# schwanbeck/YSMR

Measured on AMD Instinct MI355X. Metric: frames/sec detect+link, 1228x922 ~500 blobs, 1/2/4/8 GPU; HBM GB/s %peak, higher is better.
Workload: dtype u8 image / f32 threshold+geometry / f64 link; 1 GPU; 1228x922 stream, ~500 blobs, detect+link end to end (BASELINE configs[2], the configuration the metric is quoted on); detect_batch=248, channels=1, streams=1, parallelism=1 stream/GPU x1, tracks_alive=508, ids_issued=796

## Files before the change

ysmr_amd/csrc/batch_link.h:

```cpp
#pragma once

#include "tracker_plan.h"

constexpr unsigned BL_FLAG = 0xFFFFu, BL_SPLIT = 0xFFFEu;

constexpr int BG_THREADS = 256, BG_PER = 10;
constexpr int BG_CAND = 32;
static_assert(BG_THREADS == 4 * 64 && BL_OVF <= 64, "k_bgrid's second pass: quadrant w of overflow entry `lane` on wave w");
static_assert(BG_THREADS * BG_PER >= FUSED_MAX_DET, "k_bgrid keeps a frame's detections in registers, BG_PER per thread");

__device__ __forceinline__ void bl_rect_list(int cx, int cy, float ax, float bx, float ay, float by, float e, int G, int m, float cell,
                                             float inv, const unsigned short *start16, const float2 *xy, unsigned short *list8,
                                             unsigned short *cand)
{
    float u2 = 3.0e38f;
    int ju = 0;
    auto far2 = [&](int a, int b) {
        for (int j = a; j < b; ++j) {
            const float2 d = xy[j];
            const float dx = fmaxf(fabsf(d.x - ax), fabsf(d.x - bx)), dy = fmaxf(fabsf(d.y - ay), fabsf(d.y - by));
            const float v = dx * dx + dy * dy;
            ju = v < u2 ? j : ju;
            u2 = fminf(u2, v);
        }
    };
    for (int r = 0; r < G; ++r) {
        const int xl = max(cx - r, 0), xh = min(cx + r, G - 1);
        for (int y = max(cy - r, 0); y <= min(cy + r, G - 1); ++y) {
            if (y == cy - r || y == cy + r) far2(start16[y * G + xl], start16[y * G + xh + 1]);
            else {
                if (cx - r >= 0) far2(start16[y * G + cx - r], start16[y * G + cx - r + 1]);
                if (cx + r < G) far2(start16[y * G + cx + r], start16[y * G + cx + r + 1]);
            }
        }
        const float reach = (float)(r + 1) * cell;
        if (u2 <= reach * reach) break;
    }
    const float T = sqrtf(u2) * 1.0001f + 1.0f, T2 = T * T;
    const int rho = min((int)((T + e) * inv) + 2, G);
    int n = 0;
    for (int y = max(cy - rho, 0); y <= min(cy + rho, G - 1); ++y) {
        const int a = start16[y * G + max(cx - rho, 0)], b = start16[y * G + min(cx + rho, G - 1) + 1];
        for (int j = a; j < b; ++j) {
            const float2 d = xy[j];
            const float dx = fmaxf(fmaxf(ax - d.x, d.x - bx), 0.f), dy = fmaxf(fmaxf(ay - d.y, d.y - by), 0.f);
            if (dx * dx + dy * dy <= T2) {
                if (n < BG_CAND) cand[n * BG_THREADS] = (unsigned short)j;
                ++n;
            }
        }
    }
    int kept = 0;
    const float2 du = xy[ju];
    const float ua = ax - du.x, ub = bx - du.x, va = ay - du.y, vb = by - du.y;
    const float eps = 1.00003f, beta = 0.6f;
    const float u0 = (ua * ua + va * va) * eps + beta, u1 = (ub * ub + va * va) * eps + beta;
    const float u2c = (ua * ua + vb * vb) * eps + beta, u3 = (ub * ub + vb * vb) * eps + beta;
    if (n <= BG_CAND)
        for (int i = 0; i < n; ++i) {
            const int ji = cand[i * BG_THREADS];
            const float2 di = xy[ji];
            const float xa = ax - di.x, xb = bx - di.x, ya = ay - di.y, yb = by - di.y;
            const float s0 = xa * xa + ya * ya, s1 = xb * xb + ya * ya, s2 = xa * xa + yb * yb, s3 = xb * xb + yb * yb;
            bool beaten = ji != ju && s0 > u0 && s1 > u1 && s2 > u2c && s3 > u3;
            for (int k = 0; k < n && !beaten; k += 4) {
                float2 dk[4];
#pragma unroll
                for (int u = 0; u < 4; ++u) dk[u] = xy[cand[min(k + u, n - 1) * BG_THREADS]];
#pragma unroll
                for (int u = 0; u < 4; ++u) {
                    const float ka = ax - dk[u].x, kb = bx - dk[u].x, la = ay - dk[u].y, lb = by - dk[u].y;
                    beaten = beaten || (k + u < n && k + u != i && s0 > (ka * ka + la * la) * eps + beta && s1 > (kb * kb + la * la) * eps + beta &&
                                        s2 > (ka * ka + lb * lb) * eps + beta && s3 > (kb * kb + lb * lb) * eps + beta);
                }
            }
            if (!beaten) {
                if (kept < BL_LIST) list8[kept] = (unsigned short)ji;
                ++kept;
            }
        }
    if (n > BG_CAND || kept > BL_LIST) list8[0] = (unsigned short)BL_FLAG;
    else
        for (int k = kept; k < BL_LIST; ++k) list8[k] = (unsigned short)m;
}
__device__ __forceinline__ void bl_cell_list(int c, int G, int m, float x0, float y0, float cell, float inv, const unsigned short *start16,
                                             const float2 *xy, unsigned short *list16, unsigned short *cand)
{
    const int cx = c % G, cy = c / G;
    const float e = 4e-3f + 2e-4f * cell;
    const float ax = x0 + (float)cx * cell - e, bx = x0 + (float)(cx + 1) * cell + e;
    const float ay = y0 + (float)cy * cell - e, by = y0 + (float)(cy + 1) * cell + e;
    bl_rect_list(cx, cy, ax, bx, ay, by, e, G, m, cell, inv, start16, xy, list16 + c * BL_LIST, cand);
}
__device__ __forceinline__ void bl_quad_list(int c, int q, int G, int m, float x0, float y0, float cell, float inv, const unsigned short *start16,
                                             const float2 *xy, unsigned short *list8, unsigned short *cand)
{
    const int cx = c % G, cy = c / G;
    const float e = 4e-3f + 2e-4f * cell;
    const float hx = (float)cx + 0.5f * (float)(q & 1), hy = (float)cy + 0.5f * (float)(q >> 1);
    const float ax = x0 + hx * cell - e, bx = x0 + (hx + 0.5f) * cell + e;
    const float ay = y0 + hy * cell - e, by = y0 + (hy + 0.5f) * cell + e;
    bl_rect_list(cx, cy, ax, bx, ay, by, e, G, m, cell, inv, start16, xy, list8, cand);
}

template <bool D3>
__device__ __forceinline__ void bl_bin_frame(const float *__restrict__ det_all, const double *__restrict__ third_all,
                                             const int32_t *__restrict__ det_count, int max_det, char *grid, unsigned grid_stride)
{
    extern __shared__ __attribute__((aligned(16))) uint32_t s_out[];
    __shared__ int s_cnt[64 * 64];
    __shared__ float s_red[4][4];
    __shared__ int s_wave_sum[4];
    const int f = blockIdx.x, tid = threadIdx.x, lane = tid & 63, w = tid >> 6;
    __shared__ unsigned short s_cand[BG_CAND][BG_THREADS];
    __shared__ unsigned short s_crowded[BL_OVF];
    __shared__ int s_crowded_n;
    __shared__ int s_any_crowded;
    __shared__ int s_wide;
    const float *det = det_all + (size_t)f * max_det * 5;
    int m = det_count[f];
    m = m < 0 ? 0 : (m > max_det ? max_det : m);
    const int G = bl_grid_n(m), cells = G * G;
    unsigned short *start16 = reinterpret_cast<unsigned short *>(s_out + 16);
    float2 *xy = reinterpret_cast<float2 *>(s_out + 16 + bl_start_dwords(G));
    unsigned short *items = reinterpret_cast<unsigned short *>(s_out + 16 + bl_start_dwords(G) + 2 * bl_mp(m));
    unsigned short *list16 = reinterpret_cast<unsigned short *>(s_out + bl_list_off(m));
    float *z32 = reinterpret_cast<float *>(s_out + bl_list_off(m));
    double *z64 = nullptr;
    if constexpr (D3) z64 = reinterpret_cast<double *>(grid + (size_t)grid_stride * f + 4 * (size_t)bl3_lds_dwords_max(max_det));
    float x[BG_PER], y[BG_PER];
    double z[BG_PER];
    bool wide = false;
#pragma unroll
    for (int k = 0; k < BG_PER; ++k) {
        const int j = tid + k * BG_THREADS;
        x[k] = j < m ? det[(size_t)j * 5] : 0.f;
        y[k] = j < m ? det[(size_t)j * 5 + 1] : 0.f;
        if constexpr (D3) {
            z[k] = j < m ? (third_all + (size_t)f * max_det)[j] : 0.0;
            wide = wide || !(fabs(z[k]) < 4096.0);
        }
    }
    for (int c = tid; c < cells; c += BG_THREADS) s_cnt[c] = 0;
    if constexpr (D3) { if (tid == 0) s_wide = 0; }
    float lo_x = 3.0e38f, lo_y = 3.0e38f, hi_x = -3.0e38f, hi_y = -3.0e38f;
#pragma unroll
    for (int k = 0; k < BG_PER; ++k)
        if (tid + k * BG_THREADS < m) { lo_x = fminf(lo_x, x[k]); hi_x = fmaxf(hi_x, x[k]); lo_y = fminf(lo_y, y[k]); hi_y = fmaxf(hi_y, y[k]); }
#pragma unroll
    for (int d = 32; d >= 1; d >>= 1) {
        lo_x = fminf(lo_x, __shfl_xor(lo_x, d)); hi_x = fmaxf(hi_x, __shfl_xor(hi_x, d));
        lo_y = fminf(lo_y, __shfl_xor(lo_y, d)); hi_y = fmaxf(hi_y, __shfl_xor(hi_y, d));
    }
    if (lane == 0) { s_red[0][w] = lo_x; s_red[1][w] = hi_x; s_red[2][w] = lo_y; s_red[3][w] = hi_y; }
    __syncthreads();
    if constexpr (D3) { if (wide) s_wide = 1; }
    lo_x = s_red[0][0]; hi_x = s_red[1][0]; lo_y = s_red[2][0]; hi_y = s_red[3][0];
    for (int k = 1; k < 4; ++k) {
        lo_x = fminf(lo_x, s_red[0][k]); hi_x = fmaxf(hi_x, s_red[1][k]);
        lo_y = fminf(lo_y, s_red[2][k]); hi_y = fmaxf(hi_y, s_red[3][k]);
    }
    if (m == 0) { lo_x = lo_y = 0.f; hi_x = hi_y = 1.f; }
    const float extent = fmaxf(fmaxf(hi_x - lo_x, hi_y - lo_y), 1.0f);
    const float cell = extent / (float)(G - 2), inv = 1.0f / cell;
    const float x0 = lo_x - cell, y0 = lo_y - cell;
    if (tid < 16) s_out[tid] = 0;
    __syncthreads();
    if (tid == 0) {
        float *h = reinterpret_cast<float *>(s_out);
        h[0] = x0; h[1] = y0; h[2] = cell; h[3] = inv;
        s_out[4] = (uint32_t)G; s_out[5] = (uint32_t)m; s_out[6] = !D3 && bl_has_lists(m) ? BL_LIST : 0;
        if constexpr (D3) s_out[7] = (uint32_t)s_wide;
    }
    int cell_of[BG_PER];
#pragma unroll
    for (int k = 0; k < BG_PER; ++k) {
        int cx = (int)floorf((x[k] - x0) * inv), cy = (int)floorf((y[k] - y0) * inv);
        cx = cx < 0 ? 0 : (cx > G - 1 ? G - 1 : cx);
        cy = cy < 0 ? 0 : (cy > G - 1 ? G - 1 : cy);
        cell_of[k] = cy * G + cx;
        if (tid + k * BG_THREADS < m) atomicAdd(&s_cnt[cell_of[k]], 1);
    }
    __syncthreads();
    const int K = cells / BG_THREADS;
    int local[16], sum = 0;
#pragma unroll
    for (int k = 0; k < 16; ++k)
        if (k < K) { local[k] = sum; sum += s_cnt[tid * K + k]; }
    int incl = sum;
#pragma unroll
    for (int d = 1; d < 64; d <<= 1) { const int o = __shfl_up(incl, d); if (lane >= d) incl += o; }
    if (lane == 63) s_wave_sum[w] = incl;
    __syncthreads();
    int before = incl - sum;
    for (int k = 0; k < w; ++k) before += s_wave_sum[k];
#pragma unroll
    for (int k = 0; k < 16; ++k)
        if (k < K) {
            const int at = before + local[k];
            s_cnt[tid * K + k] = at;
            start16[tid * K + k] = (unsigned short)at;
        }
    if (tid == BG_THREADS - 1) { start16[cells] = (unsigned short)m; start16[cells + 1] = 0; }
    for (int j = m + tid; j < bl_mp(m); j += BG_THREADS) {
        xy[j] = make_float2(1.0e30f, 1.0e30f); items[j] = 0;
        if constexpr (D3) { z32[j] = 0.f; z64[j] = 0.0; }
    }
    __syncthreads();
#pragma unroll
    for (int k = 0; k < BG_PER; ++k) {
        const int j = tid + k * BG_THREADS;
        if (j < m) {
            const int at = atomicAdd(&s_cnt[cell_of[k]], 1);
            items[at] = (unsigned short)j;
            xy[at] = make_float2(x[k], y[k]);
            if constexpr (D3) { z32[at] = (float)z[k]; z64[at] = z[k]; }
        }
    }
    if (!D3 && bl_has_lists(m)) {
        for (int i = tid; i < BL_OVF * 4 * BL_LIST / 2; i += BG_THREADS) s_out[bl_ovf_off(m) + i] = 0;
        if (tid == 0) s_any_crowded = 0;
    }
    __syncthreads();
    if constexpr (!D3) {
        unsigned short *ovf16 = reinterpret_cast<unsigned short *>(s_out + bl_ovf_off(m));
        if (bl_has_lists(m) && m > 0) {
            for (int c = tid; c < cells; c += BG_THREADS) {
                bl_cell_list(c, G, m, x0, y0, cell, inv, start16, xy, list16, &s_cand[0][tid]);
                if (list16[c * BL_LIST] == BL_FLAG) s_any_crowded = 1;
            }
            __syncthreads();
        }
        if (bl_has_lists(m) && m > 0 && s_any_crowded) {
            int mine = 0;
#pragma unroll
            for (int k = 0; k < 16; ++k)
                if (k < K) mine += list16[(tid * K + k) * BL_LIST] == BL_FLAG;
            int inc2 = mine;
#pragma unroll
            for (int d = 1; d < 64; d <<= 1) { const int o = __shfl_up(inc2, d); if (lane >= d) inc2 += o; }
            if (lane == 63) s_wave_sum[w] = inc2;
            __syncthreads();
            int at = inc2 - mine;
            for (int k = 0; k < w; ++k) at += s_wave_sum[k];
            if (mine)
                for (int k = 0; k < K; ++k)
                    if (list16[(tid * K + k) * BL_LIST] == BL_FLAG) {
                        if (at < BL_OVF) s_crowded[at] = (unsigned short)(tid * K + k);
                        ++at;
                    }
            if (tid == BG_THREADS - 1) s_crowded_n = min(at, BL_OVF);
            __syncthreads();
            const int entries = s_crowded_n;
            if (lane < entries)
                bl_quad_list(s_crowded[lane], w, G, m, x0, y0, cell, inv, start16, xy, ovf16 + (4 * lane + w) * BL_LIST, &s_cand[0][tid]);
            __syncthreads();
            if (tid < entries) {
                bool fits = true;
                for (int q = 0; q < 4; ++q) fits = fits && ovf16[(4 * tid + q) * BL_LIST] != BL_FLAG;
                if (fits) reinterpret_cast<uint32_t *>(list16)[s_crowded[tid] * (BL_LIST / 2)] = BL_SPLIT | ((uint32_t)tid << 16);
            }
            __syncthreads();
        }
    }
    uint4 *out = reinterpret_cast<uint4 *>(grid + (size_t)grid_stride * f);
    const uint4 *img = reinterpret_cast<const uint4 *>(s_out);
    for (int i = tid; i < (D3 ? bl3_lds_dwords(m) : bl_grid_dwords(m)) / 4; i += BG_THREADS) out[i] = img[i];
}

__global__ __launch_bounds__(BG_THREADS) void k_bgrid(const float *__restrict__ det_all, const int32_t *__restrict__ det_count,
                                                      int max_det, char *grid, unsigned grid_stride)
{
    bl_bin_frame<false>(det_all, nullptr, det_count, max_det, grid, grid_stride);
}

struct BlSeat {
    double s0x[BL_NF], s1x[BL_NF], s0y[BL_NF], s1y[BL_NF];
    double w[BL_NF], xa[BL_NF], xb[BL_NF];
    double px, py;
    float info[3];
    int id, gone, len, mode, rank;
    bool alive;
};

__device__ __forceinline__ void bl_seat_blank(BlSeat &S)
{
#pragma unroll
    for (int f = 0; f < BL_NF; ++f) { S.s0x[f] = S.s1x[f] = S.s0y[f] = S.s1y[f] = 0.0; S.w[f] = S.xa[f] = S.xb[f] = 0.0; }
    S.px = S.py = 0.0;
    S.info[0] = S.info[1] = S.info[2] = 0.f;
    S.id = S.gone = S.len = S.mode = S.rank = 0;
    S.alive = false;
}

__device__ __forceinline__ void bl_seat_load(BlSeat &S, const BatchDev &bd, int at)
{
    const size_t sc = (size_t)bd.seat_cap;
    const double *p = bd.f64 + at;
#pragma unroll
    for (int f = 0; f < BL_NF; ++f) { S.w[f] = p[sc * f]; S.xa[f] = p[sc * (BL_NF + f)]; S.xb[f] = p[sc * (2 * BL_NF + f)]; }
    S.px = p[sc * (3 * BL_NF)];
    S.py = p[sc * (3 * BL_NF + 1)];
#pragma unroll
    for (int f = 0; f < BL_NF; ++f) {
        const double *q = p + sc * (3 * BL_NF + 2 + 4 * f);
        S.s0x[f] = q[0]; S.s1x[f] = q[sc]; S.s0y[f] = q[2 * sc]; S.s1y[f] = q[3 * sc];
    }
#pragma unroll
    for (int k = 0; k < 3; ++k) S.info[k] = bd.f32[sc * k + at];
    S.id = bd.i32[at]; S.gone = bd.i32[sc + at]; S.len = bd.i32[2 * sc + at]; S.mode = bd.i32[3 * sc + at];
    S.rank = bd.i32[4 * sc + at];
}

__device__ __forceinline__ void bl_seat_store(const BlSeat &S, const BatchDev &bd, int at)
{
    const size_t sc = (size_t)bd.seat_cap;
    double *p = bd.f64 + at;
#pragma unroll
    for (int f = 0; f < BL_NF; ++f) { p[sc * f] = S.w[f]; p[sc * (BL_NF + f)] = S.xa[f]; p[sc * (2 * BL_NF + f)] = S.xb[f]; }
    p[sc * (3 * BL_NF)] = S.px;
    p[sc * (3 * BL_NF + 1)] = S.py;
#pragma unroll
    for (int f = 0; f < BL_NF; ++f) {
        double *q = p + sc * (3 * BL_NF + 2 + 4 * f);
        q[0] = S.s0x[f]; q[sc] = S.s1x[f]; q[2 * sc] = S.s0y[f]; q[3 * sc] = S.s1y[f];
    }
#pragma unroll
    for (int k = 0; k < 3; ++k) bd.f32[sc * k + at] = S.info[k];
    bd.i32[at] = S.id; bd.i32[sc + at] = S.gone; bd.i32[2 * sc + at] = S.len; bd.i32[3 * sc + at] = S.mode;
    bd.i32[4 * sc + at] = S.rank;
}

__device__ __forceinline__ double2 bl_ring_load(const BatchDev &bd, int pos, int seat)
{
    const double *p = reinterpret_cast<const double *>(bd.ring + (size_t)pos * bd.seat_cap + seat);
    double2 v;
    v.x = __hip_atomic_load(p, __ATOMIC_RELAXED, __HIP_MEMORY_SCOPE_AGENT);
    v.y = __hip_atomic_load(p + 1, __ATOMIC_RELAXED, __HIP_MEMORY_SCOPE_AGENT);
    return v;
}
__device__ __forceinline__ double2 bl_ring_load_bytes(const BatchDev &bd, unsigned at)
{
    const double *p = reinterpret_cast<const double *>(reinterpret_cast<const char *>(bd.ring) + at);
    double2 v;
    v.x = __hip_atomic_load(p, __ATOMIC_RELAXED, __HIP_MEMORY_SCOPE_AGENT);
    v.y = __hip_atomic_load(p + 1, __ATOMIC_RELAXED, __HIP_MEMORY_SCOPE_AGENT);
    return v;
}
typedef uint32_t bl_u32x4 __attribute__((ext_vector_type(4)));
__device__ __forceinline__ bl_u32x4 bl_ring_load16(const double2 *p)
{
    bl_u32x4 v;
    asm volatile("global_load_dwordx4 %0, %1, off sc1\n\ts_waitcnt vmcnt(0)" : "=&v"(v) : "v"(p) : "memory");
    return v;
}
constexpr int BL_RING_GROUP = 3;
// ... 1653 lines not shown
```

ysmr_amd/csrc/track.hip:

```cpp
#include "common.h"
#include "set_order.h"
#include "tracker_plan.h"
#include <algorithm>
#include <cmath>
#include <cstdlib>
#include <cstring>
#include <vector>

struct DetGrid {
    const int *start;
    const int *items;
    const float *hdr;
    const float2 *xy;
};

namespace plan = tracker_plan;

struct ysmr_tracker {
    TrackerDev d;
    TrackerDev d1;
    int par = 0;
    plan::Config cfg;
    plan::Caps caps;
    int dims = 2;
// ... 1922 lines not shown
int ysmr_debug_read_bcounts(unsigned long long *out) { return (int)hipMemcpyFromSymbol(out, HIP_SYMBOL(g_bcounts), sizeof(unsigned long long) * BL_WAVES * BL_COUNTS); }
int ysmr_debug_read_bwaves(unsigned long long *out) { return (int)hipMemcpyFromSymbol(out, HIP_SYMBOL(g_bwaves), sizeof(unsigned long long) * (BL_WAVES + 1)); }
int ysmr_debug_read_bseats(unsigned long long *out) { return (int)hipMemcpyFromSymbol(out, HIP_SYMBOL(g_bseats), sizeof(unsigned long long) * 2); }
int ysmr_debug_read_brefresh(unsigned long long *out) { return (int)hipMemcpyFromSymbol(out, HIP_SYMBOL(g_brefresh), sizeof(unsigned long long) * BL_WAVES * 4); }
int ysmr_debug_read_bsteady(unsigned long long *out) { return (int)hipMemcpyFromSymbol(out, HIP_SYMBOL(g_bsteady), sizeof(unsigned long long) * BL_WAVES * 16); }
#endif

int ysmr_tracker_batched(ysmr_tracker *t) { return t && plan::is_batch(t->link()) ? 1 : 0; }

int ysmr_debug_ring_poison(ysmr_tracker *t)
{
    if (!t) return ysmr::fail(YSMR_ERR_ARG, "tracker handle is NULL");
    hipError_t e = hipDeviceSynchronize();
    int seen[2] = {0, 0};
    if (e == hipSuccess) e = hipMemcpy(seen, t->cur().n_tracks, sizeof(seen), hipMemcpyDeviceToHost);
    if (e == hipSuccess && (seen[0] != 0 || seen[1] != 0))
        return ysmr::fail(YSMR_ERR_ARG, "ysmr_debug_ring_poison is for a handle that has held no track yet");
    if (e == hipSuccess) e = hipMemset(t->bd.ring, 0xFF, sizeof(double2) * BL_HB * (size_t)t->bd.seat_cap);
    if (e == hipSuccess) e = hipDeviceSynchronize();
    return e == hipSuccess ? YSMR_OK : ysmr::fail(YSMR_ERR_HIP, "ring poison failed: %s", hipGetErrorString(e));
}
static int seat_words(ysmr_tracker *t, int (&w)[3])
{
    if (!t) return ysmr::fail(YSMR_ERR_ARG, "tracker handle is NULL");
    hipError_t e = hipDeviceSynchronize();
    if (e == hipSuccess) e = hipMemcpy(w, t->bd.head + 1, sizeof(w), hipMemcpyDeviceToHost);
    return e == hipSuccess ? YSMR_OK : ysmr::fail(YSMR_ERR_HIP, "seat words read failed: %s", hipGetErrorString(e));
}
int ysmr_debug_seat_events(ysmr_tracker *t, int *events_out, int *moved_out)
{
    int w[3];
    if (!events_out || !moved_out) return ysmr::fail(YSMR_ERR_ARG, "events_out and moved_out must be set");
    if (int rc = seat_words(t, w)) return rc;
    *events_out = w[0]; *moved_out = w[1];
    return YSMR_OK;
}
int ysmr_debug_track_waves(ysmr_tracker *t, int *out)
{
    int w[3];
    if (!out) return ysmr::fail(YSMR_ERR_ARG, "out must be set");
    if (int rc = seat_words(t, w)) return rc;
    *out = w[2];
    return YSMR_OK;
}
int ysmr_debug_ring_zero_line(ysmr_tracker *t, long long *nonzero)
{
    if (!t || !nonzero) return ysmr::fail(YSMR_ERR_ARG, "tracker handle and nonzero must be set");
    std::vector<unsigned long long> line(2 * (size_t)t->bd.seat_cap);
    hipError_t e = hipDeviceSynchronize();
    if (e == hipSuccess)
        e = hipMemcpy(line.data(), t->bd.ring + (size_t)BL_HB * t->bd.seat_cap, sizeof(double2) * (size_t)t->bd.seat_cap, hipMemcpyDeviceToHost);
    if (e != hipSuccess) return ysmr::fail(YSMR_ERR_HIP, "ring read failed: %s", hipGetErrorString(e));
    *nonzero = 0;
    for (unsigned long long w : line) *nonzero += w != 0;
    return YSMR_OK;
}

int ysmr_debug_read_grid_block(ysmr_tracker *t, int slot, int frame, void *out, size_t bytes)
{
    if (!t || !out) return ysmr::fail(YSMR_ERR_ARG, "tracker handle and out must be set");
    if (t->link() != plan::Link::batch) return ysmr::fail(YSMR_ERR_STATE, "the handle has no batch link: no grid blocks");
    if (slot < 0 || slot > 1 || t->prepared[slot].batch <= 0 || frame < 0 || frame >= t->prepared[slot].batch || bytes > t->bd.grid_stride)
        return ysmr::fail(YSMR_ERR_ARG, "slot 0 or 1 with a prepared batch, a frame of that batch, at most %u bytes", t->bd.grid_stride);
    hipError_t e = hipDeviceSynchronize();
    if (e == hipSuccess)
        e = hipMemcpy(out, t->bd.grid + ((size_t)slot * BL_MAX_BATCH + (size_t)frame) * t->bd.grid_stride, bytes, hipMemcpyDeviceToHost);
    return e == hipSuccess ? YSMR_OK : ysmr::fail(YSMR_ERR_HIP, "grid block read failed: %s", hipGetErrorString(e));
}

static BatchDev batch_dev(const ysmr_tracker *t, int block)
{
    BatchDev bd = t->bd;
    if (t->dims == 3) { bd.grid = (char *)t->grid3_block; bd.grid_stride = t->grid3_stride; }
    bd.grid += (size_t)block * BL_MAX_BATCH * bd.grid_stride;
    return bd;
}

static void bin_batch(const ysmr_tracker *t, hipStream_t st, const float *det, const double *third, const int32_t *count, int batch,
                      const BatchDev &bd)
{
    if (t->dims == 3)
        hipLaunchKernelGGL(k_bgrid3, dim3(batch), dim3(BG_THREADS), 4 * (size_t)bl3_lds_dwords_max(t->d.max_det), st, det, third, count,
                           t->d.max_det, bd.grid, bd.grid_stride);
    else
        hipLaunchKernelGGL(k_bgrid, dim3(batch), dim3(BG_THREADS), bd.grid_stride, st, det, count, t->d.max_det, bd.grid, bd.grid_stride);
}

static int tracker_prepare(ysmr_tracker *t, hipStream_t st, const float *det_dev, const double *third_dev, const int32_t *det_count_dev,
                           int batch, int slot)
{
    if (!plan::is_batch(t->link()) || batch > BL_MAX_BATCH) return YSMR_OK;
    bin_batch(t, st, det_dev, third_dev, det_count_dev, batch, batch_dev(t, slot));
    YSMR_LAUNCH_CHECK();
    t->prepared[slot] = ysmr_tracker::Prepared{det_dev, det_count_dev, third_dev, batch};
    return YSMR_OK;
}

int ysmr_tracker_prepare(ysmr_tracker *t, void *stream, const float *det_dev, const int32_t *det_count_dev, int batch, int slot)
{
    if (!t) return ysmr::fail(YSMR_ERR_ARG, "tracker handle is NULL");
    if (!det_dev || !det_count_dev || batch <= 0 || slot < 0 || slot > 1)
        return ysmr::fail(YSMR_ERR_ARG, "det_dev, det_count_dev must be set, batch > 0, slot 0 or 1");
    if (t->dims != 2) return YSMR_OK;
    return tracker_prepare(t, (hipStream_t)stream, det_dev, nullptr, det_count_dev, batch, slot);
}

int ysmr_tracker_prepare3(ysmr_tracker *t, void *stream, const float *det_dev, const double *third_dev, const int32_t *det_count_dev,
                          int batch, int slot)
{
    if (!t) return ysmr::fail(YSMR_ERR_ARG, "tracker handle is NULL");
    if (!det_dev || !third_dev || !det_count_dev || batch <= 0 || slot < 0 || slot > 1)
        return ysmr::fail(YSMR_ERR_ARG, "det_dev, third_dev, det_count_dev must be set, batch > 0, slot 0 or 1");
    if (t->dims != 3) return ysmr::fail(YSMR_ERR_STATE, "ysmr_tracker_prepare3 needs a 3-D handle (ysmr_tracker_dimensions)");
    return tracker_prepare(t, (hipStream_t)stream, det_dev, third_dev, det_count_dev, batch, slot);
}

static int tracker_update(ysmr_tracker *t, hipStream_t st, const void *det_dev, int det_is_f64, const double *third_dev, int m,
                          const int32_t *m_dev, int32_t frame_index, ysmr_row *rows_dev, int32_t *n_rows_dev, int32_t *claim_col_dev,
                          int32_t *n_before_dev, int32_t *new_cols_dev, int32_t *n_new_dev)
{
    if (int rc = state_to_std(t, st)) return rc;
    FrameArgs a;
    a.det = det_dev; a.f64 = det_is_f64 != 0; a.third = third_dev;
    a.m = m; a.m_dev = m_dev; a.frame = frame_index;
    a.rows = rows_dev; a.rows_capacity = t->d.capacity;
    a.n_rows = n_rows_dev; a.claim = claim_col_dev; a.n_before = n_before_dev; a.new_cols = new_cols_dev; a.n_new = n_new_dev;
    return launch_frame(t, st, a);
}

int ysmr_tracker_update(ysmr_tracker *t, void *stream, const void *det_dev, int det_is_f64, int m,
                        const int32_t *m_dev, int32_t frame_index, ysmr_row *rows_dev, int32_t *n_rows_dev,
                        int32_t *claim_col_dev, int32_t *n_before_dev, int32_t *new_cols_dev, int32_t *n_new_dev)
{
    if (!t) return ysmr::fail(YSMR_ERR_ARG, "tracker handle is NULL");
    if (m < 0 && !m_dev) return ysmr::fail(YSMR_ERR_ARG, "m < 0 requires m_dev");
    if (m > t->d.max_det) return ysmr::fail(YSMR_ERR_CAPACITY, "m = %d exceeds max_det = %d", m, t->d.max_det);
    if (!det_dev && m != 0) return ysmr::fail(YSMR_ERR_ARG, "det_dev is NULL");
    if (t->dims != 2) return ysmr::fail(YSMR_ERR_STATE, "a 3-D handle is updated with ysmr_tracker_update3");
    return tracker_update(t, (hipStream_t)stream, det_dev, det_is_f64, nullptr, m, m_dev, frame_index, rows_dev, n_rows_dev,
                          claim_col_dev, n_before_dev, new_cols_dev, n_new_dev);
}

int ysmr_tracker_update3(ysmr_tracker *t, void *stream, const void *det_dev, int det_is_f64, const double *third_dev, int m,
                         const int32_t *m_dev, int32_t frame_index, ysmr_row *rows_dev, int32_t *n_rows_dev,
                         int32_t *claim_col_dev, int32_t *n_before_dev, int32_t *new_cols_dev, int32_t *n_new_dev)
{
    if (!t) return ysmr::fail(YSMR_ERR_ARG, "tracker handle is NULL");
    if (m < 0 && !m_dev) return ysmr::fail(YSMR_ERR_ARG, "m < 0 requires m_dev");
    if (m > t->d.max_det) return ysmr::fail(YSMR_ERR_CAPACITY, "m = %d exceeds max_det = %d", m, t->d.max_det);
    if ((!det_dev || !third_dev) && m != 0) return ysmr::fail(YSMR_ERR_ARG, "det_dev / third_dev is NULL");
    if (t->dims != 3) return ysmr::fail(YSMR_ERR_STATE, "ysmr_tracker_update3 needs a 3-D handle (ysmr_tracker_dimensions)");
    return tracker_update(t, (hipStream_t)stream, det_dev, det_is_f64, third_dev, m, m_dev, frame_index, rows_dev, n_rows_dev,
                          claim_col_dev, n_before_dev, new_cols_dev, n_new_dev);
}

static int tracker_run(ysmr_tracker *t, hipStream_t st, const float *det_dev, const double *third_dev, const int32_t *det_count_dev,
                       int batch, int32_t first_frame_index, ysmr_row *rows_dev, long long rows_capacity, long long *row_count_dev)
{
    const bool d3 = t->dims == 3;
    const size_t md = (size_t)t->d.max_det;
    t->linked = true;
    if (plan::is_batch(t->link())) {
        if (int rc = state_to_batch(t, st)) return rc;
        for (int f0 = 0; f0 < batch; f0 += BL_MAX_BATCH) {
            const int nb = std::min(batch - f0, BL_MAX_BATCH);
            const float *det = det_dev + (size_t)f0 * md * 5;
            const double *third = d3 ? third_dev + (size_t)f0 * md : nullptr;
            int block = 2;
// ... 129 lines not shown
```

ysmr_amd/csrc/tracker_plan.h:

```cpp
#pragma once
#include <cmath>
#include <cstddef>
#include <cstdint>
#include <cstring>
#include <vector>

#include "hd.h"

#ifndef __HIPCC__
struct alignas(16) double2 { double x, y; };
#endif

#define YSMR_MAX_FILTERS 8

struct TrackerDev {
    int *n_tracks, *next_id, *err, *n_free;
    int *order, *gone;
    int *row_arg;
    double *row_min;
    long long *row_base;
    int capacity, max_det, n_f, use_gsff, hist_cap, table_cap, gain_total, gone_by_row;
    int gains_decoupled;
    double max_gone, lik_min;
    int n_i[YSMR_MAX_FILTERS];
// ... 13 lines not shown
    int *set_table;
    unsigned long long *link_key;
    int *link_row;
    int *link_claim;
    int *claim_slot;
    int *claim_row;
};

#ifndef YSMR_BL_THREADS
#define YSMR_BL_THREADS 768
#endif
constexpr int BL_THREADS = YSMR_BL_THREADS;
constexpr int BL_WAVES = BL_THREADS / 64;
constexpr int BL_HB = 32;
constexpr int BL_NF = 3;
#ifndef YSMR_BL_MAX_BATCH
#define YSMR_BL_MAX_BATCH 256
#endif
constexpr int BL_MAX_BATCH = YSMR_BL_MAX_BATCH;
constexpr int BL_TABLE = 4096;
constexpr int BL_SF64 = 3 * BL_NF + 2 + 4 * BL_NF;
constexpr int BL_REFRESH = 64;

struct BatchDev {
    double2 *ring;
    double *f64;
    float *f32;
    int *i32;
    int *head;
    char *grid;
    unsigned grid_stride;
    int seat_cap;
};

struct BlGains { double alpha[BL_NF][2], beta[BL_NF][2]; };
constexpr int GRID_N = 128;
constexpr int GRID_CELLS = GRID_N * GRID_N;
YSMR_HD inline size_t grid_bytes_per_frame(int max_det)
{
    return (sizeof(int) * (GRID_CELLS + 64) + sizeof(int) * (size_t)max_det + 64 + 2 * sizeof(float) * (size_t)max_det + 255) / 256 * 256;
}

constexpr int FRAME_THREADS = 256;
constexpr int FRAME_TABLE = 4096;
YSMR_HD inline size_t frame_lds_bytes(int cap, int max_det, int gain_total)
{
    return 8 * ((size_t)gain_total + max_det) + 4 * ((size_t)max_det + 2 * (size_t)cap + 16) + 2 * 2 * FRAME_TABLE + 64;
}

constexpr int TRACKER_MAX_SIZE = 65536;
constexpr int FUSED_MAX_DET = 2456;
constexpr size_t FRAME_LDS_LIMIT = 150 * 1024;
constexpr double FUSED_MAX_GONE = 32000.0;
constexpr size_t LINK_LDS_LIMIT = 140 * 1024;
constexpr size_t BL_LDS_LIMIT = 160 * 1024;

constexpr int BL_LIST = 8;
constexpr int BL_OVF = 8;
YSMR_HD inline int bl_grid_n(int m) { return m <= 128 ? 16 : (m <= 600 ? 32 : (m <= 1300 ? 48 : 64)); }
YSMR_HD inline bool bl_has_lists(int m) { return bl_grid_n(m) <= 32; }
YSMR_HD inline int bl_start_dwords(int G) { return ((G * G + 2) / 2 + 3) / 4 * 4; }
YSMR_HD inline int bl_pad8(int m) { return (m + 7) / 8 * 8; }
YSMR_HD inline int bl_mp(int m) { return bl_pad8(m + 1); }
YSMR_HD inline int bl_list_off(int m)
{
    return 16 + bl_start_dwords(bl_grid_n(m)) + 2 * bl_mp(m) + bl_mp(m) / 2;
}
YSMR_HD inline int bl_ovf_off(int m)
{
    return bl_list_off(m) + bl_grid_n(m) * bl_grid_n(m) * BL_LIST / 2;
}
YSMR_HD inline int bl_grid_dwords(int m)
{
    const int raw = bl_has_lists(m) ? bl_ovf_off(m) + BL_OVF * 4 * BL_LIST / 2 : bl_list_off(m);
    return (raw + 255) / 256 * 256;
}
YSMR_HD inline int bl_grid_dwords_max(int max_det)
{
    int most = bl_grid_dwords(max_det);
    const int steps[4] = {128, 600, 1300, max_det};
    for (int k = 0; k < 4; ++k)
        if (steps[k] <= max_det && bl_grid_dwords(steps[k]) > most) most = bl_grid_dwords(steps[k]);
    return most;
}

struct BlShared {
    int cnt[BL_MAX_BATCH];
    int used[2];
    int n_dead[2];
    int tie[2];
    int dead_id[2][BL_THREADS];
    int wave_cnt[2][BL_WAVES];
    int set_state[2];
    int top;
    long long rows_then;
};

YSMR_HD inline int bl_md_padded(int max_det) { return (max_det + 3) / 4 * 4; }
YSMR_HD inline size_t bl_lds_bytes(int max_det)
{
    return 2 * 4 * (size_t)bl_grid_dwords_max(max_det) + (3 * 8 + 4) * (size_t)bl_md_padded(max_det) + 4 * BL_TABLE + 64;
}
YSMR_HD inline size_t bl_lds_total(int max_det) { return bl_lds_bytes(max_det) + (sizeof(BlShared) + 15) / 16 * 16; }

YSMR_HD inline int bl3_lds_dwords(int m) { return (bl_list_off(m) + bl_mp(m) + 255) / 256 * 256; }
YSMR_HD inline int bl3_lds_dwords_max(int max_det) { return bl3_lds_dwords(max_det); }
YSMR_HD inline size_t bl3_grid_stride(int max_det)
{
    return 4 * (size_t)bl3_lds_dwords_max(max_det) + (8 * (size_t)bl_mp(max_det) + 1023) / 1024 * 1024;
}
YSMR_HD inline size_t bl3_lds_bytes(int max_det)
{
    return 2 * 4 * (size_t)bl3_lds_dwords_max(max_det) + (3 * 8 + 4) * (size_t)bl_md_padded(max_det) + 4 * BL_TABLE + 64;
}
YSMR_HD inline size_t bl3_lds_total(int max_det) { return bl3_lds_bytes(max_det) + (sizeof(BlShared) + 15) / 16 * 16; }

namespace tracker_plan {

enum class Bad { none, size, filters, fps, horizons, horizon_max };
struct Status {
    Bad what = Bad::none;
    int a = 0, b = 0, c = 0;
    double x = 0.0;
    explicit operator bool() const { return what != Bad::none; }
};

inline Status horizons(double fps, int n_min, double n_max, int n_f, int *n_i)
{
    if (n_f < 1 || n_f > YSMR_MAX_FILTERS) return Status{Bad::filters, YSMR_MAX_FILTERS, n_f};
    if (!(fps > 0)) return Status{Bad::fps};
    double top = n_max > 0 ? n_max : fps;
    double p = (top - n_min) / n_f;
    for (int i = 1; i <= n_f; ++i) n_i[i - 1] = (int)(n_min + p * i);
    for (int i = 0; i < n_f; ++i)
        if (n_i[i] < 1 || (i && n_i[i] <= n_i[i - 1])) return Status{Bad::horizons, n_min, n_f, 0, top};
    return Status{};
}

inline void closed_form_gain(int N, double *g)
{
    double st2 = 0.0;
    for (int j = 0; j < N; ++j) { double tj = j - (N - 1) / 2.0; st2 += tj * tj; }
    std::memset(g, 0, sizeof(double) * 4 * N);
    for (int j = 0; j < N; ++j) {
        double tj = j - (N - 1) / 2.0;
        double c = 1.0 / N + (st2 > 0 ? tj * ((N + 1) / 2.0) / st2 : 0.0);
        g[2 * j] = c;
        g[2 * N + 2 * j + 1] = c;
    }
}

struct Config {
    int capacity, max_det, use_gsff;
    double max_gone;
    int n_f, n_i[YSMR_MAX_FILTERS], gain_off[YSMR_MAX_FILTERS], gain_total;
    int hist_cap, table_cap, rec_stride;
    int gains_decoupled;
    bool gains_affine;
    BlGains bgains;
};

inline Status configure(double max_disappeared, double fps, int n_min, double n_max, int n_f, int use_gsff, int capacity,
                        int max_det, const double *gains, Config &c, std::vector<double> &gains_out)
{
    if (capacity <= 0 || max_det <= 0 || capacity > TRACKER_MAX_SIZE || max_det > TRACKER_MAX_SIZE)
        return Status{Bad::size, capacity, max_det};
// ... 164 lines not shown
```

Before: 293,100 frames/s.

## Split grid binning into bin, per-cell list, and crowded-split kernels

The single per-frame binning kernel used to also build per-cell candidate lists and quadrant overflow lists inside one 256-thread block. This moves list building into k_blist, which launches several blocks per frame (one per 256 cells, with launch bounds allowing four blocks per CU), and moves the crowded-cell quadrant split into k_bsplit, which exits early when no cell is flagged. The aim is more parallelism and less LDS per block than the monolithic kernel allowed. In exchange there are two extra launches per batch and a round trip of the frame's grid through global memory, and the groups and LDS sizes are capped at the m=600 configuration.

Result: no change. 293,600 frames/s, median of 2 (+0.2%).

```diff
diff --git a/ysmr_amd/csrc/batch_link.h b/ysmr_amd/csrc/batch_link.h
--- a/ysmr_amd/csrc/batch_link.h
+++ b/ysmr_amd/csrc/batch_link.h
@@ -6,7 +6,7 @@
 
 constexpr int BG_THREADS = 256, BG_PER = 10;
 constexpr int BG_CAND = 32;
-static_assert(BG_THREADS == 4 * 64 && BL_OVF <= 64, "k_bgrid's second pass: quadrant w of overflow entry `lane` on wave w");
+static_assert(BG_THREADS == 4 * 64 && BL_OVF <= 64, "k_bsplit, the second pass: quadrant w of overflow entry `lane` on wave w");
 static_assert(BG_THREADS * BG_PER >= FUSED_MAX_DET, "k_bgrid keeps a frame's detections in registers, BG_PER per thread");
 
 __device__ __forceinline__ void bl_rect_list(int cx, int cy, float ax, float bx, float ay, float by, float e, int G, int m, float cell,
@@ -84,13 +84,13 @@
         for (int k = kept; k < BL_LIST; ++k) list8[k] = (unsigned short)m;
 }
 __device__ __forceinline__ void bl_cell_list(int c, int G, int m, float x0, float y0, float cell, float inv, const unsigned short *start16,
-                                             const float2 *xy, unsigned short *list16, unsigned short *cand)
+                                             const float2 *xy, unsigned short *list8, unsigned short *cand)
 {
     const int cx = c % G, cy = c / G;
     const float e = 4e-3f + 2e-4f * cell;
     const float ax = x0 + (float)cx * cell - e, bx = x0 + (float)(cx + 1) * cell + e;
     const float ay = y0 + (float)cy * cell - e, by = y0 + (float)(cy + 1) * cell + e;
-    bl_rect_list(cx, cy, ax, bx, ay, by, e, G, m, cell, inv, start16, xy, list16 + c * BL_LIST, cand);
+    bl_rect_list(cx, cy, ax, bx, ay, by, e, G, m, cell, inv, start16, xy, list8, cand);
 }
 __device__ __forceinline__ void bl_quad_list(int c, int q, int G, int m, float x0, float y0, float cell, float inv, const unsigned short *start16,
                                              const float2 *xy, unsigned short *list8, unsigned short *cand)
@@ -112,10 +112,6 @@
     __shared__ float s_red[4][4];
     __shared__ int s_wave_sum[4];
     const int f = blockIdx.x, tid = threadIdx.x, lane = tid & 63, w = tid >> 6;
-    __shared__ unsigned short s_cand[BG_CAND][BG_THREADS];
-    __shared__ unsigned short s_crowded[BL_OVF];
-    __shared__ int s_crowded_n;
-    __shared__ int s_any_crowded;
     __shared__ int s_wide;
     const float *det = det_all + (size_t)f * max_det * 5;
     int m = det_count[f];
@@ -124,7 +120,6 @@
     unsigned short *start16 = reinterpret_cast<unsigned short *>(s_out + 16);
     float2 *xy = reinterpret_cast<float2 *>(s_out + 16 + bl_start_dwords(G));
     unsigned short *items = reinterpret_cast<unsigned short *>(s_out + 16 + bl_start_dwords(G) + 2 * bl_mp(m));
-    unsigned short *list16 = reinterpret_cast<unsigned short *>(s_out + bl_list_off(m));
     float *z32 = reinterpret_cast<float *>(s_out + bl_list_off(m));
     double *z64 = nullptr;
     if constexpr (D3) z64 = reinterpret_cast<double *>(grid + (size_t)grid_stride * f + 4 * (size_t)bl3_lds_dwords_max(max_det));
@@ -217,61 +212,107 @@
             if constexpr (D3) { z32[at] = (float)z[k]; z64[at] = z[k]; }
         }
     }
-    if (!D3 && bl_has_lists(m)) {
-        for (int i = tid; i < BL_OVF * 4 * BL_LIST / 2; i += BG_THREADS) s_out[bl_ovf_off(m) + i] = 0;
-        if (tid == 0) s_any_crowded = 0;
-    }
     __syncthreads();
-    if constexpr (!D3) {
-        unsigned short *ovf16 = reinterpret_cast<unsigned short *>(s_out + bl_ovf_off(m));
-        if (bl_has_lists(m) && m > 0) {
-            for (int c = tid; c < cells; c += BG_THREADS) {
-                bl_cell_list(c, G, m, x0, y0, cell, inv, start16, xy, list16, &s_cand[0][tid]);
-                if (list16[c * BL_LIST] == BL_FLAG) s_any_crowded = 1;
-            }
-            __syncthreads();
-        }
-        if (bl_has_lists(m) && m > 0 && s_any_crowded) {
-            int mine = 0;
-#pragma unroll
-            for (int k = 0; k < 16; ++k)
-                if (k < K) mine += list16[(tid * K + k) * BL_LIST] == BL_FLAG;
-            int inc2 = mine;
-#pragma unroll
-            for (int d = 1; d < 64; d <<= 1) { const int o = __shfl_up(inc2, d); if (lane >= d) inc2 += o; }
-            if (lane == 63) s_wave_sum[w] = inc2;
-            __syncthreads();
-            int at = inc2 - mine;
-            for (int k = 0; k < w; ++k) at += s_wave_sum[k];
-            if (mine)
-                for (int k = 0; k < K; ++k)
-                    if (list16[(tid * K + k) * BL_LIST] == BL_FLAG) {
-                        if (at < BL_OVF) s_crowded[at] = (unsigned short)(tid * K + k);
-                        ++at;
-                    }
-            if (tid == BG_THREADS - 1) s_crowded_n = min(at, BL_OVF);
-            __syncthreads();
-            const int entries = s_crowded_n;
-            if (lane < entries)
-                bl_quad_list(s_crowded[lane], w, G, m, x0, y0, cell, inv, start16, xy, ovf16 + (4 * lane + w) * BL_LIST, &s_cand[0][tid]);
-            __syncthreads();
-            if (tid < entries) {
-                bool fits = true;
-                for (int q = 0; q < 4; ++q) fits = fits && ovf16[(4 * tid + q) * BL_LIST] != BL_FLAG;
-                if (fits) reinterpret_cast<uint32_t *>(list16)[s_crowded[tid] * (BL_LIST / 2)] = BL_SPLIT | ((uint32_t)tid << 16);
-            }
-            __syncthreads();
-        }
-    }
     uint4 *out = reinterpret_cast<uint4 *>(grid + (size_t)grid_stride * f);
     const uint4 *img = reinterpret_cast<const uint4 *>(s_out);
-    for (int i = tid; i < (D3 ? bl3_lds_dwords(m) : bl_grid_dwords(m)) / 4; i += BG_THREADS) out[i] = img[i];
+    if constexpr (D3) {
+        for (int i = tid; i < bl3_lds_dwords(m) / 4; i += BG_THREADS) out[i] = img[i];
+    } else if (bl_has_lists(m)) {
+        for (int i = tid; i < bl_list_off(m) / 4; i += BG_THREADS) out[i] = img[i];
+        for (int i = bl_ovf_off(m) / 4 + tid; i < bl_grid_dwords(m) / 4; i += BG_THREADS) out[i] = make_uint4(0, 0, 0, 0);
+    } else {
+        for (int i = tid; i < bl_grid_dwords(m) / 4; i += BG_THREADS) out[i] = img[i];
+    }
 }
 
 __global__ __launch_bounds__(BG_THREADS) void k_bgrid(const float *__restrict__ det_all, const int32_t *__restrict__ det_count,
                                                       int max_det, char *grid, unsigned grid_stride)
 {
     bl_bin_frame<false>(det_all, nullptr, det_count, max_det, grid, grid_stride);
+}
+
+static_assert(BL_LIST_THREADS == BG_THREADS && BL_LIST_SCRATCH == 2 * BG_CAND + 2 * BL_LIST, "tracker_plan.h sizes k_blist's LDS");
+
+__device__ __forceinline__ void bl_list_frame_in(const char *block, int m, uint32_t *s_in)
+{
+    const uint4 *src = reinterpret_cast<const uint4 *>(block);
+    uint4 *dst = reinterpret_cast<uint4 *>(s_in);
+    for (int i = threadIdx.x; i < bl_list_frame_dwords(m) / 4; i += BG_THREADS) dst[i] = src[i];
+    __syncthreads();
+}
+
+__global__ __launch_bounds__(BG_THREADS, 4) void k_blist(const int32_t *__restrict__ det_count, int max_det, int groups, char *grid,
+                                                         unsigned grid_stride)
+{
+    extern __shared__ __attribute__((aligned(16))) uint32_t s_in[];
+    __shared__ unsigned short s_cand[BG_CAND][BG_THREADS];
+    __shared__ __attribute__((aligned(16))) unsigned short s_slot[BG_THREADS][BL_LIST];
+    const int f = blockIdx.x / groups, p = blockIdx.x % groups, tid = threadIdx.x;
+    int m = det_count[f];
+    m = m < 0 ? 0 : (m > max_det ? max_det : m);
+    const int G = bl_grid_n(m);
+    if (!bl_has_lists(m) || m == 0 || p * BG_THREADS >= G * G) return;
+    char *block = grid + (size_t)grid_stride * f;
+    bl_list_frame_in(block, m, s_in);
+    const float *h = reinterpret_cast<const float *>(s_in);
+    const unsigned short *start16 = reinterpret_cast<const unsigned short *>(s_in + 16);
+    const float2 *xy = reinterpret_cast<const float2 *>(s_in + 16 + bl_start_dwords(G));
+    const int c = p * BG_THREADS + tid;
+    bl_cell_list(c, G, m, h[0], h[1], h[2], h[3], start16, xy, s_slot[tid], &s_cand[0][tid]);
+    reinterpret_cast<uint4 *>(block + 4 * (size_t)bl_list_off(m))[c] = *reinterpret_cast<const uint4 *>(s_slot[tid]);
+}
+
+__global__ __launch_bounds__(BG_THREADS) void k_bsplit(const int32_t *__restrict__ det_count, int max_det, char *grid, unsigned grid_stride)
+{
+    extern __shared__ __attribute__((aligned(16))) uint32_t s_in[];
+    __shared__ unsigned short s_cand[BG_CAND][BG_THREADS];
+    __shared__ __attribute__((aligned(16))) unsigned short s_ovf[BL_OVF * 4][BL_LIST];
+    __shared__ unsigned short s_crowded[BL_OVF];
+    __shared__ int s_crowded_n;
+    __shared__ int s_wave_sum[4];
+    const int f = blockIdx.x, tid = threadIdx.x, lane = tid & 63, w = tid >> 6;
+    int m = det_count[f];
+    m = m < 0 ? 0 : (m > max_det ? max_det : m);
+    if (!bl_has_lists(m) || m == 0) return;
+    const int G = bl_grid_n(m), K = G * G / BG_THREADS;
+    char *block = grid + (size_t)grid_stride * f;
+    unsigned short *list16 = reinterpret_cast<unsigned short *>(block + 4 * (size_t)bl_list_off(m));
+    unsigned flags = 0;
+#pragma unroll
+    for (int k = 0; k < 4; ++k)
+        if (k < K) flags |= (unsigned)(list16[(tid * K + k) * BL_LIST] == BL_FLAG) << k;
+    if (!__syncthreads_or((int)flags)) return;
+    for (int i = tid; i < BL_OVF * 4 * BL_LIST / 2; i += BG_THREADS) reinterpret_cast<uint32_t *>(&s_ovf[0][0])[i] = 0;
+    bl_list_frame_in(block, m, s_in);
+    const float *h = reinterpret_cast<const float *>(s_in);
+    const float x0 = h[0], y0 = h[1], cell = h[2], inv = h[3];
+    const unsigned short *start16 = reinterpret_cast<const unsigned short *>(s_in + 16);
+    const float2 *xy = reinterpret_cast<const float2 *>(s_in + 16 + bl_start_dwords(G));
+    const int mine = __popc(flags);
+    int inc2 = mine;
+#pragma unroll
+    for (int d = 1; d < 64; d <<= 1) { const int o = __shfl_up(inc2, d); if (lane >= d) inc2 += o; }
+    if (lane == 63) s_wave_sum[w] = inc2;
+    __syncthreads();
+    int at = inc2 - mine;
+    for (int k = 0; k < w; ++k) at += s_wave_sum[k];
+    if (mine)
+        for (int k = 0; k < K; ++k)
+            if (flags >> k & 1) {
+                if (at < BL_OVF) s_crowded[at] = (unsigned short)(tid * K + k);
+                ++at;
+            }
+    if (tid == BG_THREADS - 1) s_crowded_n = min(at, BL_OVF);
+    __syncthreads();
+    const int entries = s_crowded_n;
+    if (lane < entries) bl_quad_list(s_crowded[lane], w, G, m, x0, y0, cell, inv, start16, xy, s_ovf[4 * lane + w], &s_cand[0][tid]);
+    __syncthreads();
+    if (tid < entries) {
+        bool fits = true;
+        for (int q = 0; q < 4; ++q) fits = fits && s_ovf[4 * tid + q][0] != BL_FLAG;
+        if (fits) reinterpret_cast<uint32_t *>(list16)[s_crowded[tid] * (BL_LIST / 2)] = BL_SPLIT | ((uint32_t)tid << 16);
+    }
+    if (tid < 4 * entries) reinterpret_cast<uint4 *>(block + 4 * (size_t)bl_ovf_off(m))[tid] = *reinterpret_cast<const uint4 *>(s_ovf[tid]);
 }
 
 struct BlSeat {
diff --git a/ysmr_amd/csrc/track.hip b/ysmr_amd/csrc/track.hip
--- a/ysmr_amd/csrc/track.hip
+++ b/ysmr_amd/csrc/track.hip
@@ -2028,8 +2028,13 @@
     if (t->dims == 3)
         hipLaunchKernelGGL(k_bgrid3, dim3(batch), dim3(BG_THREADS), 4 * (size_t)bl3_lds_dwords_max(t->d.max_det), st, det, third, count,
                            t->d.max_det, bd.grid, bd.grid_stride);
-    else
-        hipLaunchKernelGGL(k_bgrid, dim3(batch), dim3(BG_THREADS), bd.grid_stride, st, det, count, t->d.max_det, bd.grid, bd.grid_stride);
+    else {
+        const int md = t->d.max_det, groups = bl_list_groups_max(md);
+        const size_t frame_lds = 4 * (size_t)bl_list_frame_dwords_max(md);
+        hipLaunchKernelGGL(k_bgrid, dim3(batch), dim3(BG_THREADS), 4 * (size_t)bl_bin_dwords_max(md), st, det, count, md, bd.grid, bd.grid_stride);
+        hipLaunchKernelGGL(k_blist, dim3(batch * groups), dim3(BG_THREADS), frame_lds, st, count, md, groups, bd.grid, bd.grid_stride);
+        hipLaunchKernelGGL(k_bsplit, dim3(batch), dim3(BG_THREADS), frame_lds, st, count, md, bd.grid, bd.grid_stride);
+    }
 }
 
 static int tracker_prepare(ysmr_tracker *t, hipStream_t st, const float *det_dev, const double *third_dev, const int32_t *det_count_dev,
diff --git a/ysmr_amd/csrc/tracker_plan.h b/ysmr_amd/csrc/tracker_plan.h
--- a/ysmr_amd/csrc/tracker_plan.h
+++ b/ysmr_amd/csrc/tracker_plan.h
@@ -119,6 +119,18 @@
     for (int k = 0; k < 4; ++k)
         if (steps[k] <= max_det && bl_grid_dwords(steps[k]) > most) most = bl_grid_dwords(steps[k]);
     return most;
+}
+YSMR_HD inline int bl_bin_dwords_max(int max_det) { return (bl_list_off(max_det) + 255) / 256 * 256; }
+constexpr int BL_LIST_THREADS = 256;
+constexpr int BL_LIST_SCRATCH = 32 * 2 + BL_LIST * 2;
+YSMR_HD inline int bl_list_groups(int m) { return bl_has_lists(m) ? (bl_grid_n(m) * bl_grid_n(m) + BL_LIST_THREADS - 1) / BL_LIST_THREADS : 0; }
+YSMR_HD inline int bl_list_groups_max(int max_det) { return bl_list_groups(max_det < 600 ? max_det : 600); }
+YSMR_HD inline int bl_list_frame_dwords(int m) { return 16 + bl_start_dwords(bl_grid_n(m)) + 2 * bl_mp(m); }
+YSMR_HD inline int bl_list_frame_dwords_max(int max_det) { return bl_list_frame_dwords(max_det < 600 ? max_det : 600); }
+constexpr size_t BL_LIST_LDS_LIMIT = BL_LDS_LIMIT / 4;
+YSMR_HD inline size_t bl_list_lds_bytes(int m)
+{
+    return bl_has_lists(m) ? 4 * (size_t)bl_list_frame_dwords(m) + (size_t)BL_LIST_SCRATCH * BL_LIST_THREADS : 0;
 }
 
 struct BlShared {
```
